# CIS565-Fall-2017/Project3-CUDA-Path-Tracer

Hardware: AMD Instinct MI355X
Metric: Mrays/sec (live paths x bounces) at 800x800 Cornell depth 8 (higher is better)
Workload: dtype f32

## Files before the change

project3-cuda-path-tracer_amd/csrc/pt_h_api.hpp:

```cpp
#pragma once

namespace one {

const char *pt_last_error(void) { return g_err; }
const char *pt_version(void) {
#ifdef PT_EXPERIMENTS
    return "ptmi355 0.1 (gfx950, fp32 no-contract, wave64) +experiments";
#else
    return "ptmi355 0.1 (gfx950, fp32 no-contract, wave64)";
#endif
}

void pt_free(void) {
    if (!R.live && !R.scratch) return;
    if (R.stream) (void)hipStreamSynchronize(R.stream);
    for (int k = 0; k < OV_MAX_LANES; ++k) {
        if (R.lane[k].stream) (void)hipStreamSynchronize(R.lane[k].stream);
        if (R.lane[k].la_stream) (void)hipStreamSynchronize(R.lane[k].la_stream);
    }
    if (R.la_gstream) (void)hipStreamSynchronize(R.la_gstream);
    for (int k = 0; k < 2; ++k) if (R.pool_mem[k]) (void)hipFree(R.pool_mem[k]);
    if (R.isect_mem) (void)hipFree(R.isect_mem);
    if (R.sort_table) (void)hipFree(R.sort_table);
    if (R.cache_mem) (void)hipFree(R.cache_mem);
    if (R.state_mem) (void)hipFree(R.state_mem);
    if (R.state_ended) (void)hipFree(R.state_ended);
    if (R.final_mem) (void)hipFree(R.final_mem);
    if (R.image && R.own_image) (void)hipFree(R.image);
    if (R.d_geoms) (void)hipFree(R.d_geoms);
    if (R.d_mats) (void)hipFree(R.d_mats);
    if (R.d_tris) (void)hipFree(R.d_tris);
    if (R.d_cull) (void)hipFree(R.d_cull);
    if (R.d_grec) (void)hipFree(R.d_grec);
    if (R.d_tri_bound) (void)hipFree(R.d_tri_bound);
    if (R.d_ginfo) (void)hipFree(R.d_ginfo);
    if (R.d_env) (void)hipFree(R.d_env);
    if (R.d_lights) (void)hipFree(R.d_lights);
    if (R.tex.d_texels) (void)hipFree(R.tex.d_texels);
    if (R.tex.d_tab) (void)hipFree(R.tex.d_tab);
    if (R.bump.d_texels) (void)hipFree(R.bump.d_texels);
    if (R.bump.d_tab) (void)hipFree(R.bump.d_tab);
    if (R.d_vnormals) (void)hipFree(R.d_vnormals);
    if (R.mesh_hit) (void)hipFree(R.mesh_hit);
    for (int k = 0; k < 2; ++k) if (R.mesh_flags[k]) (void)hipFree(R.mesh_flags[k]);
    if (R.d_bvh_nodes) (void)hipFree(R.d_bvh_nodes);
    if (R.d_bvh_meshes) (void)hipFree(R.d_bvh_meshes);
    if (R.d_bvh_tris) (void)hipFree(R.d_bvh_tris);
    if (R.d_bvh_top) (void)hipFree(R.d_bvh_top);
    if (R.d_cam_mask) (void)hipFree(R.d_cam_mask);
    R.d_cam_mask = nullptr; R.cam_mask_valid = false;
    if (R.d_cull0) (void)hipFree(R.d_cull0);
    R.d_cull0 = nullptr; R.cull0_tiles = 0;
    free_lanes();
    if (R.ctl) (void)hipFree(R.ctl);
    if (R.dir_mem) (void)hipFree(R.dir_mem);
// ... 155 lines not shown
    if (const char *wm = getenv("PTMI355_WHOLE_MAX_HOST")) R.whole_max_host_paths = strtoull(wm, nullptr, 10);
    if (getenv("PTMI355_WHOLE_MAX") && !getenv("PTMI355_WHOLE_MAX_HOST")) R.whole_max_host_paths = R.whole_max_paths;
    if (const char *e = getenv("PTMI355_OVERLAP")) {
        const int nl = atoi(e);
        R.ov_enabled = nl != 0;
        if (nl >= 2) { R.ov_lanes = std::min(nl, OV_MAX_LANES); R.ov_lanes_set = true; }
    }
    if (const char *e = getenv("PTMI355_OVERLAP_GB")) R.ov_budget_gb = atof(e);
    if (const char *e = pt_experiment("PTMI355_LANE_STREAMS")) R.ov_streams = std::max(1, atoi(e));
    R.epi_enabled = true;
    if (const char *e = pt_experiment("PTMI355_HOST_EPILOGUE")) R.epi_enabled = atoi(e) != 0;
    if (d->flags & PT_MOMENTS) R.epi_enabled = false;
    if (const char *e = pt_experiment("PTMI355_EPI_DIRECT")) R.epi_direct_enabled = atoi(e) != 0;
    R.defer_enabled = true;
    if (const char *e = pt_experiment("PTMI355_DEFER_DIR")) R.defer_enabled = atoi(e) != 0;
    R.own_enabled = true;
    if (const char *e = pt_experiment("PTMI355_OWN_SURFACE")) R.own_enabled = atoi(e) != 0;
    R.first_hit_enabled = true;
    if (const char *e = pt_experiment("PTMI355_FIRST_HIT")) R.first_hit_enabled = atoi(e) != 0;
    R.first_two_enabled = true;
    if (const char *e = pt_experiment("PTMI355_FIRST_TWO")) R.first_two_enabled = atoi(e) != 0;
    R.first_state_enabled = true;
    if (const char *e = pt_experiment("PTMI355_FIRST_STATE")) R.first_state_enabled = atoi(e) != 0;
    R.host_sparse_enabled = (d->flags & (PT_HOST_SPARSE | PT_SHARED_IMAGE)) != 0;
    if (const char *e = pt_experiment("PTMI355_ASYNC_DIRECT")) R.async_direct_enabled = atoi(e) != 0;
    R.pin_enabled = true;
    if (const char *e = pt_experiment("PTMI355_PIN")) R.pin_enabled = atoi(e) != 0;
    R.npix = W * H;
    R.map.W = W; R.map.H = H; R.map.tile_index = d->tile_index; R.map.tile_count = tile_count;
    R.map.strip_rows = tile_count > 1 ? d->strip_rows : H;
    R.map.tile_pixels = tile_rows(d->tile_index, tile_count, R.map.strip_rows, H) * W;
    if (R.map.tile_pixels <= 0) return fail(PT_ERR_INVALID, "pt_init: tile owns no rows");
    make_div_magic((uint32_t)R.map.tile_pixels, &R.map.div_magic, &R.map.div_shift);
    auto magic_holds = [](uint32_t d, uint32_t magic, uint32_t shift) {
        auto fast = [&](uint32_t n) {
            if (d == 1) return n;
            const uint32_t q = (uint32_t)(((uint64_t)magic * n) >> 32);
            return (((n - q) >> 1) + q) >> shift;
        };
        for (uint64_t k = 0; k <= 0xffffffffull / d && k < 4096; ++k)
            for (int e = -1; e <= 1; ++e) {
                const uint64_t n = k * d + (uint64_t)(int64_t)e;
                if (n <= 0xffffffffull && fast((uint32_t)n) != (uint32_t)n / d) return false;
            }
        const uint32_t probes[] = {0u, 1u, d - 1, d, d + 1, 0x7fffffffu, 0x80000000u, 0xfffffffeu, 0xffffffffu};
        for (uint32_t n : probes)
// ... 86 lines not shown
        if (d->num_materials >= (1 << 28)) return fail(PT_ERR_INVALID, "pt_init: at most 2^28 materials");
        HIPCHK(hipMalloc(&R.d_grec, gath.size() * 4));
        HIPCHK(hipMalloc((void **)&R.d_ginfo, ginfo.size() * 4));
        HIPCHK(hipMemcpy(R.d_grec, gath.data(), gath.size() * 4, hipMemcpyHostToDevice));
        HIPCHK(hipMemcpy(R.d_ginfo, ginfo.data(), ginfo.size() * 4, hipMemcpyHostToDevice));
        if (d->num_geoms > 0) {
            hipLaunchKernelGGL(k_face_normals, dim3((d->num_geoms * 8 + BLOCK - 1) / BLOCK), dim3(BLOCK), 0, R.stream,
                               R.d_grec, (const uint32_t *)R.d_ginfo, d->num_geoms);
            HIPCHK(hipGetLastError());
            HIPCHK(hipStreamSynchronize(R.stream));
        }
        R.scene.grec = R.d_grec; R.scene.ginfo = R.d_ginfo;
    }
    R.mesh_mode = MESH_NONE;
    for (int i = 0; i < d->num_geoms; ++i)
        if (d->geoms[i].type == PT_TRIANGLE_MESH) R.mesh_mode = (d->flags & PT_MESH_BVH) ? MESH_BVH : MESH_TILES;
    R.geoms_keep.assign(d->geoms, d->geoms + d->num_geoms);
    if (d->num_triangles > 0) R.tris_keep.assign(d->triangles, d->triangles + d->num_triangles);
    R.desc.geoms = R.geoms_keep.data();
    R.desc.triangles = R.tris_keep.empty() ? nullptr : R.tris_keep.data();
    if (d->num_meshes > 0) R.meshes_keep.assign(d->meshes, d->meshes + d->num_meshes);
    R.desc.meshes = R.meshes_keep.empty() ? nullptr : R.meshes_keep.data();
    R.grec_frames.assign((size_t)std::max(1, d->num_geoms) * 4, 0.0f);
    {
        const int rc = upload_cull(&R.desc, R.cam);
        if (rc != PT_OK) return rc;
    }
    if (R.mesh_mode == MESH_BVH) {
        const int rc = upload_bvh(&R.desc, grec);
        if (rc != PT_OK) return rc;
        HIPCHK(hipMemcpy(R.d_geoms, grec.data(), grec.size() * 4, hipMemcpyHostToDevice));
    }
    R.grec_keep = grec;
    {
        const size_t base = ((size_t)LDS_CTL_WORDS + (size_t)WAVES * PW_WORDS) * 4 +
                            (R.mesh_mode == MESH_TILES ? (size_t)WAVES * TRQ_WORDS * 4 : 0);
        const size_t scene = (size_t)scene_lds_words(d->num_materials, d->num_geoms) * 4;
        R.scene_lds = base + scene <= 32 * 1024;
        if (const char *e = getenv("PTMI355_SCENE_LDS")) R.scene_lds = atoi(e) != 0 && base + scene <= 64 * 1024;
        R.lds_bytes = base + (R.scene_lds ? scene : 0);
        R.lds_bytes = (R.lds_bytes + 15) & ~(size_t)15;
        if (const char *pad = pt_experiment("PTMI355_LDS_PAD")) R.lds_bytes += (size_t)atoi(pad);
    }

    R.sort_keys = 0;
    if ((R.flags & PT_SORT_MATERIAL) && (R.flags & PT_COMPACT) && !(R.flags & (PT_UNFUSED | PT_FAKE_SHADER | PT_CACHE_FIRST)) &&
// ... 60 lines not shown
    HIPCHK(hipMalloc((void **)&R.persist, sizeof(Persist)));
    HIPCHK(hipMemsetAsync(R.persist, 0, sizeof(Persist), R.stream));
    hipDeviceProp_t prop;
    HIPCHK(hipGetDeviceProperties(&prop, d->device));
    const int cus = prop.multiProcessorCount > 0 ? prop.multiProcessorCount : 256;
    int per_cu = 8;
    {
        const bool sorted = R.sort_keys > 0;
        const bool own = R.mesh_mode == MESH_NONE && !sorted;
        auto size_for = [&](auto sh) -> int {
            constexpr int SH = decltype(sh)::value;
            constexpr int SHN = SH & ~SH_SMOOTH;
            const void *fns[2];
            if (R.mesh_mode == MESH_BVH) { fns[0] = bounce_fn<MESH_PRE, SH>(R.scene_lds, false, false); fns[1] = bounce_fn<MESH_PRE, SH>(R.scene_lds, true, false); }
            else if (R.mesh_mode == MESH_TILES) { fns[0] = bounce_fn<MESH_TILES, SH>(R.scene_lds, false, sorted); fns[1] = bounce_fn<MESH_TILES, SH>(R.scene_lds, true, sorted); }
            else { fns[0] = bounce_fn<MESH_NONE, SHN>(R.scene_lds, false, sorted); fns[1] = bounce_fn<MESH_NONE, SHN>(R.scene_lds, true, sorted); }
            const void *fns_own[2] = {own ? bounce_fn<MESH_NONE, SHN>(R.scene_lds, false, false, true) : fns[0], own ? bounce_fn<MESH_NONE, SHN>(R.scene_lds, true, false, true) : fns[1]};
            const void *fns_tab[4] = {own ? bounce_fn<MESH_NONE, SHN>(R.scene_lds, false, false, false, true) : fns[0], own ? bounce_fn<MESH_NONE, SHN>(R.scene_lds, true, false, false, true) : fns[1],
                                      own ? bounce_fn<MESH_NONE, SHN>(R.scene_lds, false, false, true, true) : fns[0], own ? bounce_fn<MESH_NONE, SHN>(R.scene_lds, true, false, true, true) : fns[1]};
            const void *fns_two[2] = {own ? bounce_fn<MESH_NONE, SHN>(R.scene_lds, true, false, false, true, true) : fns[0],
                                      own ? bounce_fn<MESH_NONE, SHN>(R.scene_lds, true, false, true, true, true) : fns[0]};
            const void *fns_state[2] = {own ? bounce_fn<MESH_NONE, SHN>(R.scene_lds, true, false, false, true, true, true) : fns[0],
                                        own ? bounce_fn<MESH_NONE, SHN>(R.scene_lds, true, false, true, true, true, true) : fns[0]};
            for (const void *f : {fns[0], fns[1], fns_own[0], fns_own[1], fns_tab[0], fns_tab[1], fns_tab[2], fns_tab[3], fns_two[0], fns_two[1],
                                  fns_state[0], fns_state[1]}) {
                int n = 0;
                HIPCHK(hipOccupancyMaxActiveBlocksPerMultiprocessor(&n, f, BLOCK, R.lds_bytes));
                per_cu = std::min(per_cu, n);
            }
            return PT_OK;
        };
        int rc = size_for(std::integral_constant<int, 0>{});
        if (rc == PT_OK && (R.nlights > 0 || sky_session())) rc = size_for(std::integral_constant<int, SH_DIRECT>{});
        if (rc == PT_OK && (R.flags & PT_TEXTURES) && !(R.flags & PT_FAKE_SHADER)) rc = size_for(std::integral_constant<int, SH_TEX>{});
        if (rc == PT_OK && (R.flags & PT_SMOOTH_NORMALS) && !(R.flags & PT_FAKE_SHADER) && R.mesh_mode != MESH_NONE)
            rc = size_for(std::integral_constant<int, SH_SMOOTH>{});
        if (rc != PT_OK) return rc;
    }
    if (per_cu < 1) per_cu = 1;
    if (per_cu > 8) per_cu = 8;
    if (const char *e = pt_experiment("PTMI355_WGS_PER_CU")) per_cu = std::max(1, std::min(per_cu, atoi(e)));
    R.grid = (int)std::min<uint32_t>((R.max_tiles + WAVES - 1) / WAVES, (uint32_t)cus * (uint32_t)per_cu);
    R.per_cu = per_cu;
    if (const char *e = pt_experiment("PTMI355_LA_CUS")) R.la_cus = std::max(0, std::min(64, atoi(e) & ~7));
    if (R.grid < 1) R.grid = 1;
    if (R.grid * WAVES > 8192) R.grid = 8192 / WAVES;
    {
        int n = 0;
// ... 724 lines not shown
```

project3-cuda-path-tracer_amd/csrc/pt_h_enqueue.hpp:

```cpp
#pragma once

namespace {

BounceArgs bounce_args(int depth) {
    BounceArgs a{};
    a.dbg_counts = R.dbg_counts;
    a.in = R.pool[R.cur];
    a.out = (R.flags & PT_COMPACT) ? R.pool[R.cur ^ 1] : R.pool[R.cur];
    a.isect = R.isect;
    a.scene = R.scene;
    a.map = R.map;
    a.ctl = R.ctl;
    a.dir_in = tile_dir((R.flags & PT_COMPACT) ? R.cur_dir : -1);
    a.dir_out = tile_dir(depth);
    a.fin = R.final_mem;
    a.fin_stamp = R.fin_serial;
    a.cam = R.cam;
    a.lens = R.lens;
    a.depth = depth; a.trace_depth = R.trace_depth; a.iter0 = R.step_iter0;
    a.pool_n = (uint32_t)R.map.tile_pixels * (uint32_t)R.step_count;
    a.gen_rays = (depth == 0 && R.gen_fused) ? 1 : 0;
    a.mesh_hit = R.mesh_hit;
    a.mesh_flags_in = R.mesh_flags[depth & 1]; a.mesh_flags_out = R.mesh_flags[(depth + 1) & 1];
    a.mesh_scan = R.mesh_marked ? 0 : 1;
// ... 64 lines not shown
            if (R.mesh_mode == MESH_BVH) { constexpr int MESH = MESH_BVH; CALL; }            \
            else if (R.mesh_mode == MESH_TILES) { constexpr int MESH = MESH_TILES; CALL; }   \
            else { constexpr int MESH = MESH_NONE; CALL; }              \
        }                                                               \
    } while (0)

void launch_intersect(const Pool &in, const uint32_t *n_ptr, uint32_t n_fixed, const RangeDir &dir,
                      const uint32_t *nprev, bool raygen_pool = false, bool generate = false) {
    const bool same_rays = !R.lens.aa && !(R.lens.radius > 0.0f);
    const unsigned long long *cull0 = (raygen_pool && R.cull0_tiles && same_rays) ? R.d_cull0 : nullptr;
    RayGen gen{};
    if (generate) {
        gen.cam = R.cam; gen.lens = R.lens; gen.map = R.map; gen.trace_depth = R.trace_depth;
        gen.iter0 = R.step_iter0;
        PT_MESH_DISPATCH(hipLaunchKernelGGL((k_intersect<MESH, SLDS, true>), dim3(R.grid), dim3(BLOCK), R.lds_bytes, R.stream, in,
                                            R.isect, R.scene, n_ptr, n_fixed, dir, nprev, R.ctl, cull0, R.cull0_tiles, gen));
        return;
    }
    PT_MESH_DISPATCH(hipLaunchKernelGGL((k_intersect<MESH, SLDS>), dim3(R.grid), dim3(BLOCK), R.lds_bytes, R.stream, in,
                                        R.isect, R.scene, n_ptr, n_fixed, dir, nprev, R.ctl, cull0, R.cull0_tiles, gen));
}

template <int MESH, int SH = 0>
const void *bounce_fn(bool slds, bool gen, bool sorted, bool own = false, bool table = false, bool first2 = false, bool state2 = false) {
    if constexpr (MESH == MESH_NONE) {
        if (table && !sorted) {
            constexpr int SH0 = SH & (SH_ENV | SH_GLOSSY);
            if (first2 && state2) {
                if (own) return slds ? (const void *)k_bounce<MODE_STATE2, true, MESH, true, true, false, true, 0> : (const void *)k_bounce<MODE_STATE2, true, MESH, false, true, false, true, 0>;
                return slds ? (const void *)k_bounce<MODE_STATE2, true, MESH, true, true, false, false, 0> : (const void *)k_bounce<MODE_STATE2, true, MESH, false, true, false, false, 0>;
            }
            if (first2) {
                if (own) return slds ? (const void *)k_bounce<MODE_FIRST2, true, MESH, true, true, false, true, SH0> : (const void *)k_bounce<MODE_FIRST2, true, MESH, false, true, false, true, SH0>;
                return slds ? (const void *)k_bounce<MODE_FIRST2, true, MESH, true, true, false, false, SH0> : (const void *)k_bounce<MODE_FIRST2, true, MESH, false, true, false, false, SH0>;
            }
            if (own) {
                if (slds) return gen ? (const void *)k_bounce<MODE_CACHE0, true, MESH, true, true, false, true, SH0> : (const void *)k_bounce<MODE_CACHE0, true, MESH, true, false, false, true, SH0>;
                return gen ? (const void *)k_bounce<MODE_CACHE0, true, MESH, false, true, false, true, SH0> : (const void *)k_bounce<MODE_CACHE0, true, MESH, false, false, false, true, SH0>;
            }
            if (slds) return gen ? (const void *)k_bounce<MODE_CACHE0, true, MESH, true, true, false, false, SH0> : (const void *)k_bounce<MODE_CACHE0, true, MESH, true, false, false, false, SH0>;
            return gen ? (const void *)k_bounce<MODE_CACHE0, true, MESH, false, true, false, false, SH0> : (const void *)k_bounce<MODE_CACHE0, true, MESH, false, false, false, false, SH0>;
        }
        if (own && !sorted) {
            if (slds) return gen ? (const void *)k_bounce<MODE_FUSED, true, MESH, true, true, false, true, SH> : (const void *)k_bounce<MODE_FUSED, true, MESH, true, false, false, true, SH>;
            return gen ? (const void *)k_bounce<MODE_FUSED, true, MESH, false, true, false, true, SH> : (const void *)k_bounce<MODE_FUSED, true, MESH, false, false, false, true, SH>;
        }
    }
    if constexpr (MESH != MESH_PRE) {
// ... 124 lines not shown
        R.sorted_isects = true;
        R.step_depth = depth + 1;
        return PT_OK;
    }
    const bool same_rays = !R.lens.aa && !(R.lens.radius > 0.0f);
    const bool auto0 = depth == 0 && !unfused && R.first_hit_enabled && R.cache_mem != nullptr && !(R.flags & PT_FAKE_SHADER) &&
                       R.mesh_mode == MESH_NONE && R.sort_keys == 0 && same_rays && a.tex_tab == nullptr &&
                       !(a.nlights > 0 && depth >= a.trace_depth - 1);
    const bool cached0 = depth == 0 && !unfused && ((R.flags & PT_CACHE_FIRST) || auto0);
    const bool first2 = may_fuse && auto0 && !(R.flags & PT_CACHE_FIRST) && compact && R.gen_fused && R.first_two_enabled &&
                        R.trace_depth >= 2 && !(a.nlights > 0 && 1 >= a.trace_depth - 1);
    const bool state2 = first2 && R.state_mem != nullptr && a.env_n == 0;
    if (first2) {
        depth = 1;
        a.depth = 1;
        a.dir_out = tile_dir(1);
        a.gen_rays = 1;
    }
    a.defer_dir = (compact && !unfused && R.mesh_mode == MESH_NONE && R.sort_keys == 0 && depth + 1 < R.trace_depth &&
                   R.defer_enabled) ? 1 : 0;
    R.own_form = own_surface_plan((uint64_t)a.pool_n, R.scene.ngeoms,
                                  compact && !unfused && R.mesh_mode == MESH_NONE && R.sort_keys == 0 &&
                                  R.own_enabled);
    if (cached0 && !R.cache_valid) {
        StageTimer tm(PT_STAGE_INTERSECT);
        const Isect cache{R.cache_mem, (uint32_t)R.map.tile_pixels};
        const int blocks = std::min(R.grid, (R.map.tile_pixels + BLOCK - 1) / BLOCK);
        const hipStream_t fs = R.lane_cur ? R.lane_main : R.stream;
        PT_MESH_DISPATCH(hipLaunchKernelGGL((k_cache_first<MESH, SLDS>), dim3(blocks), dim3(BLOCK), R.lds_bytes, fs,
                                            cache, R.scene, R.cam, R.map, R.state_mem, R.state_ended));
        HIPCHK(hipGetLastError());
        if (R.lane_cur) {
            HIPCHK(hipEventRecord(R.ov_enter, fs));
            HIPCHK(hipStreamWaitEvent(R.stream, R.ov_enter, 0));
            R.first_hit_refence = true;
        }
        R.cache_valid = true;
        R.first_hit_fills++;
    }
    if (!cached0 && !unfused && R.mesh_mode == MESH_BVH) {
        StageTimer tm(PT_STAGE_MESH);
        if (compact) hipLaunchKernelGGL((k_mesh<true>), dim3(R.grid_mesh), dim3(MESH_BLOCK), MESH_LDS_BYTES, R.stream, a);
        else hipLaunchKernelGGL((k_mesh<false>), dim3(R.grid_mesh), dim3(MESH_BLOCK), MESH_LDS_BYTES, R.stream, a);
        HIPCHK(hipGetLastError());
    }
    StageTimer tm(PT_STAGE_BOUNCE);
    if (cached0) {
        a.isect = Isect{R.cache_mem, (uint32_t)R.map.tile_pixels};
        R.first_hit_launches++;
        if (state2) {
            a.first_state = R.state_mem; a.first_ended = R.state_ended; a.first_ended_tiles = (uint32_t)(R.map.tile_pixels / TILE);
            R.first_two_launches++; R.first_state_launches++; tm.two_bounces(); launch_bounce<MODE_STATE2, true>(a);
        }
        else if (first2) { R.first_two_launches++; tm.two_bounces(); launch_bounce<MODE_FIRST2, true>(a); }
        else if (compact) launch_bounce<MODE_CACHE0, true>(a); else launch_bounce<MODE_CACHE0, false>(a);
    } else if (unfused) {
        if (compact) launch_bounce<MODE_ISECT, true>(a); else launch_bounce<MODE_ISECT, false>(a);
    } else {
        if (compact) launch_bounce<MODE_FUSED, true>(a); else launch_bounce<MODE_FUSED, false>(a);
    }
    HIPCHK(hipGetLastError());
    if (R.mesh_mode == MESH_BVH) {
        R.mesh_marked = !cached0 && !unfused;
    }
    if (compact) { R.cur ^= 1; R.cur_dir = depth; }
    R.pool_own = R.own_form;
    R.step_depth = depth + 1;
    return PT_OK;
}

int enqueue_fake(void) {
    const uint32_t total = (uint32_t)R.map.tile_pixels * (uint32_t)R.step_count;
    launch_intersect(R.pool[R.cur], nullptr, total, tile_dir(-1), nullptr);
    HIPCHK(hipGetLastError());
    hipLaunchKernelGGL(k_shade_fake, dim3((total + BLOCK - 1) / BLOCK), dim3(BLOCK), 0, R.stream, R.pool[R.cur],
                       R.isect, R.scene.mats, R.map, R.step_iter0, total, R.final_mem, R.fin_serial);
    HIPCHK(hipGetLastError());
    R.step_depth = 1;
    return PT_OK;
}
// ... 270 lines not shown
```

project3-cuda-path-tracer_amd/csrc/pt_h_scene.hpp:

```cpp
#pragma once

namespace {

int upload_tri_bounds(const pt_scene_desc *d, double Rorigin);

int upload_cull(const pt_scene_desc *d, const pt_camera &cam) {
    const int n = d->num_geoms;
    std::vector<const float *> inv((size_t)std::max(1, n));
    std::vector<char> sph((size_t)std::max(1, n)), skip((size_t)std::max(1, n));
    for (int i = 0; i < n; ++i) {
        inv[(size_t)i] = &d->geoms[i].inverseTransform.m[0][0];
        sph[(size_t)i] = d->geoms[i].type == PT_SPHERE;
        skip[(size_t)i] = d->geoms[i].type == PT_TRIANGLE_MESH;
    }
    const double eye[3] = {(double)cam.position.x, (double)cam.position.y, (double)cam.position.z};
    std::vector<ptcull::Box> boxes;
    std::vector<double> pts(eye, eye + 3);
    for (int t = 0; t < d->num_triangles; ++t) {
        const pt_vec3 *v = &d->triangles[t].v0;
        double m = 0.0;
        for (int k = 0; k < 3; ++k) m = std::max(m, (double)std::fabs(v[k].x) + std::fabs(v[k].y) + std::fabs(v[k].z));
        if (t == 0 || m > pts[3]) { if (pts.size() < 6) pts.resize(6, 0.0); pts[3] = m; pts[4] = 0.0; pts[5] = 0.0; }
    }
    R.scene.rmax = ptcull::make_boxes(inv.data(), reinterpret_cast<const bool *>(sph.data()),
                                      reinterpret_cast<const bool *>(skip.data()), n, pts.data(), (int)(pts.size() / 3), boxes);
    std::vector<float> rec((size_t)std::max(1, n) * CULL_WORDS, 0.0f);
    for (int i = 0; i < n; ++i) {
        float *r = rec.data() + (size_t)i * CULL_WORDS;
        for (int k = 0; k < 3; ++k) ptcull::centre_half(boxes[(size_t)i].lo[k], boxes[(size_t)i].hi[k], r[2 * k], r[2 * k + 1]);
        int ax = 3;
        if (d->geoms[i].type == PT_CUBE && !pt_experiment("PTMI355_NO_AXIS_REJECT"))
            ax = ptcull::reject_row(&d->geoms[i].inverseTransform.m[0][0], &r[7]);
        if (ax == 4 && pt_experiment("PTMI355_NO_ROW_REJECT")) ax = 3;
        const int tw = d->geoms[i].type | (ax << 8);
        memcpy(&r[6], &tw, 4);
        const uint32_t ent = ((uint32_t)d->geoms[i].type << 7) | ((uint32_t)i << 9);
        memcpy(&r[11], &ent, 4);
    }
    if (!R.d_cull) HIPCHK(hipMalloc(&R.d_cull, rec.size() * 4));
    HIPCHK(hipMemcpyAsync(R.d_cull, rec.data(), rec.size() * 4, hipMemcpyHostToDevice, R.stream));
    HIPCHK(hipStreamSynchronize(R.stream));
    R.scene.cull = R.d_cull;
    R.cull_eye_reach = std::fabs(eye[0]) + std::fabs(eye[1]) + std::fabs(eye[2]);
    return upload_tri_bounds(d, (double)R.scene.rmax);
}

void make_tri_bounds(const pt_triangle *tris, int count, double Rorigin, float *out) {
    const double u = 0x1p-24;
    const float pad = ptbvh::spec_pad(reinterpret_cast<const float *>(tris), count);
    const int n4 = (count + 3) & ~3;
    for (int i = 0; i < n4; ++i) {
        float *o = out + (size_t)i * 4;
        if (i >= count) { o[0] = o[1] = o[2] = 0.0f; o[3] = -1.0f; continue; }
        const pt_triangle &t = tris[i];
        const float v0[3] = {t.v0.x, t.v0.y, t.v0.z};
        const float e1[3] = {t.v1.x - t.v0.x, t.v1.y - t.v0.y, t.v1.z - t.v0.z};
        const float e2[3] = {t.v2.x - t.v0.x, t.v2.y - t.v0.y, t.v2.z - t.v0.z};
        double c[3], h2 = 0.0, cinf = 0.0;
        bool fin = true;
        for (int a = 0; a < 3; ++a) {
            const float x1 = v0[a] + e1[a], x2 = v0[a] + e2[a];
            const float lo = std::fmin(v0[a], std::fmin(x1, x2)) - pad, hi = std::fmax(v0[a], std::fmax(x1, x2)) + pad;
            if (!std::isfinite(lo) || !std::isfinite(hi)) fin = false;
// ... 235 lines not shown
```

project3-cuda-path-tracer_amd/csrc/pt_h_session.hpp:

```cpp
#pragma once

namespace {

constexpr size_t ERR_BYTES = 512;
char g_err[ERR_BYTES] = "";
thread_local char *t_err = g_err;

int fail(int code, const char *fmt, ...) {
    va_list ap;
    va_start(ap, fmt);
    vsnprintf(t_err, ERR_BYTES, fmt, ap);
    va_end(ap);
    return code;
}

#define HIPCHK(expr)                                                                            \
    do {                                                                                        \
        hipError_t e_ = (expr);                                                                 \
        if (e_ != hipSuccess)                                                                   \
            return fail(PT_ERR_DEVICE, "HIP error (%s:%d): %s: %s", __builtin_strrchr(__FILE__, '/') ? __builtin_strrchr(__FILE__, '/') + 1 : __FILE__, __LINE__, #expr, \
                        hipGetErrorString(e_));                                                 \
    } while (0)

template <class Texel> struct CubeMaps {
// ... 13 lines not shown
    uint32_t flags = 0;
    int device = 0;
    hipStream_t stream = nullptr;
    bool own_stream = false;
    TileMap map{};
    int npix = 0;
    uint32_t cap = 0;
    int max_batch = 1;
    float *pool_mem[2] = {nullptr, nullptr};
    Pool pool[2]{};
    int cur = 0;
    float *isect_mem = nullptr;
    uint32_t *sort_table = nullptr;
    float *cache_mem = nullptr;
    bool cache_valid = false;
    bool first_hit_enabled = true;
    bool first_hit_refence = false;
    bool first_two_enabled = true;
    uint64_t first_two_launches = 0;
    float *state_mem = nullptr;
    uint32_t *state_ended = nullptr;
    bool first_state_enabled = true;
    uint64_t first_state_launches = 0;
    uint64_t first_hit_fills = 0, first_hit_launches = 0;
    Isect isect{};
    float *final_mem = nullptr;
    uint32_t fin_serial = 0;
    float *image = nullptr;
    bool own_image = false;
    float *d_geoms = nullptr, *d_mats = nullptr, *d_tris = nullptr;
    float *d_cull = nullptr, *d_grec = nullptr;
    float *d_tri_bound = nullptr;
    size_t tri_bound_words = 0;
    std::vector<float> grec_frames;
    uint32_t *d_ginfo = nullptr;
    double cull_eye_reach = 0.0;
    std::vector<pt_geom> geoms_keep;
    std::vector<pt_triangle> tris_keep;
    std::vector<pt_mesh> meshes_keep;
    std::vector<float> grec_keep;
    bool scene_lds = true;
    SceneDev scene{};
    float4 *d_env = nullptr;
    int env_n = 0;
    std::vector<float> env_keep;
    float *d_lights = nullptr;
// ... 249 lines not shown
```

project3-cuda-path-tracer_amd/csrc/pt_k_bounce.hpp:

```cpp
#pragma once

namespace {

enum { MODE_FUSED = 0, MODE_ISECT = 1, MODE_CACHE0 = 2, MODE_FIRST2 = 3, MODE_STATE2 = 4 };
constexpr bool mode_first2(int mode) { return mode == MODE_FIRST2 || mode == MODE_STATE2; }

template <typename T>
__device__ __forceinline__ T karg_field(size_t offset) {
    const __attribute__((address_space(4))) char *kp = (const __attribute__((address_space(4))) char *)__builtin_amdgcn_kernarg_segment_ptr();
    asm volatile("" : "+s"(kp));
    return *(const __attribute__((address_space(4))) T *)(kp + offset);
}
template <typename T>
__device__ __forceinline__ T karg_struct(size_t offset) {
    static_assert(sizeof(T) % 4 == 0, "whole dwords");
    const __attribute__((address_space(4))) char *kp = (const __attribute__((address_space(4))) char *)__builtin_amdgcn_kernarg_segment_ptr();
    asm volatile("" : "+s"(kp));
    uint32_t w[sizeof(T) / 4];
#pragma unroll
    for (size_t k = 0; k < sizeof(T) / 4; ++k) w[k] = *(const __attribute__((address_space(4))) uint32_t *)(kp + offset + 4 * k);
    T t;
    __builtin_memcpy(&t, w, sizeof(T));
    return t;
}
// ... 511 lines not shown
        asm volatile("s_waitcnt vmcnt(0)" ::: "memory");
        __syncthreads();
        if (threadIdx.x == 0) {
            const bool last = elect_last(a.ctl->bucket[a.depth][0], &a.ctl->done[a.depth]);
            if (last) {
                __builtin_amdgcn_fence(__ATOMIC_ACQUIRE, "agent");
                asm volatile("s_waitcnt vmcnt(0)" ::: "memory");
            }
            sctl[0] = last ? 1u : 0u;
        }
        __syncthreads();
        STAMP(7);
        if (sctl[0]) {
            const unsigned long long t0 = __builtin_amdgcn_s_memrealtime();
            scan_range_counts(a.dir_out, &a.ctl->nlive[a.depth + 1], sctl + 16, R * TILE, PT_ALIGNED_TILES && !SORT);
            if (threadIdx.x == 0) a.ctl->scan_ticks[a.depth] = (uint32_t)(__builtin_amdgcn_s_memrealtime() - t0);
#ifdef PT_STAMPS
            if (threadIdx.x == 0 && a.depth == PT_STAMPS) { a.ctl->stamp[8] = t0; a.ctl->stamp[9] = __builtin_amdgcn_s_memrealtime(); }
#endif
        }
    }
}

__device__ __forceinline__ void fold_iter_counts(const uint32_t *counts, uint32_t G, int depth, Control *ctl, Persist *per, HostStats *hs,
                                                 uint32_t iterations, uint32_t serial, uint32_t *lds ) {
    constexpr int PER_PASS = BLOCK / 32;
    unsigned long long rays = 0;
    uint32_t first = 0;
    for (int d0 = 0; d0 < depth; d0 += PER_PASS) {
        const int d = d0 + (int)(threadIdx.x >> 5);
        uint32_t sum = 0;
        if (d < depth)
            for (uint32_t b = threadIdx.x & 31u; b < G; b += 32u)
                sum += __hip_atomic_load(&counts[(uint32_t)d * G + b], __ATOMIC_RELAXED, __HIP_MEMORY_SCOPE_AGENT);
        for (int off = 16; off > 0; off >>= 1) sum += __shfl_down(sum, off, 32);
        if ((threadIdx.x & 31u) == 0) lds[threadIdx.x >> 5] = sum;
        __syncthreads();
        if (threadIdx.x == 0)
            for (int k = 0; k < PER_PASS && d0 + k < depth; ++k) {
                const uint32_t tot = lds[k];
                ctl->alive[d0 + k] = tot;
                if (hs) hs->alive[d0 + k] = tot;
                rays += tot;
                if (d0 + k == 0) first = tot;
            }
        __syncthreads();
// ... 134 lines not shown
```

project3-cuda-path-tracer_amd/csrc/pt_types.hpp:

```cpp
#pragma once

namespace {


#ifndef PT_MIN_WAVES
#define PT_MIN_WAVES 4
#endif
#ifndef PT_FUSED_WAVES
#define PT_FUSED_WAVES 6
#endif
#ifndef PT_ISECT_WAVES
#define PT_ISECT_WAVES 4
#endif
#ifndef PT_PRE_WAVES
#define PT_PRE_WAVES 6
#endif
#ifndef PT_ITER_WAVES
#define PT_ITER_WAVES PT_MIN_WAVES
#endif
#ifndef PT_SORT_WAVES
#define PT_SORT_WAVES 6
#endif
#ifndef PT_LOOP_WAVES
#define PT_LOOP_WAVES 3
// ... 203 lines not shown
    const unsigned long long *cam_mask;
    const unsigned long long *cull0;
    uint32_t cull0_tiles;
    float *epi_image, *epi_host;
    int epi_direct;
    uint32_t *iter_counts;
    Persist *persist;
    HostStats *host_stats;
    uint32_t *sort_table;
    int nbins;
    int defer_dir;
    const float4 *env;
    int env_n;
    const float *lights;
    int nlights;
    const float4 *tex;
    const int2 *tex_tab;
    const ptd::bump_texel *bumps;
    const int2 *bump_tab;
    float *first_state;
    const uint32_t *first_ended;
    uint32_t first_ended_tiles;
    const float *vnormals;
};

enum : uint32_t { FS_ZERO = 0, FS_CONST = 1, FS_DIFFUSE = 2, FS_FIXED = 3, FS_KIND_MASK = 3 };
__host__ __device__ constexpr size_t first_state_bytes(size_t tile_pixels) { return ((tile_pixels + 63) / 64) * 2560; }

enum : int {
    SH_ENV = 1,
    SH_GLOSSY = 2,
    SH_DIRECT = 4,
    SH_TEX = 8,
    SH_SMOOTH = 16
};

struct RayGen {
    pt_camera cam;
    Lens lens;
    TileMap map;
    int trace_depth, iter0;
};

__device__ __forceinline__ int local_to_pixel(const TileMap &m, int j) {
    if (m.tile_count == 1) return j;
    int ly = j / m.W;
    int x = j - ly * m.W;
// ... 38 lines not shown
```

project3-cuda-path-tracer_amd/csrc/ptmi355.hip:

```cpp
#include <hip/hip_runtime.h>

#include <algorithm>
#include <atomic>
#include <cfloat>
#include <cmath>
#include <cstdarg>
#include <cstdio>
#include <cstdlib>
#include <cstring>
#include <type_traits>
#include <vector>

#include "../../include/ptmi355.h"
#include "pt_device.hpp"

static_assert(sizeof(pt_vec3) == 12 && sizeof(pt_mat4) == 64 && sizeof(pt_ray) == 24, "ABI");
static_assert(sizeof(pt_geom) == 236 && offsetof(pt_geom, transform) == 44 &&
              offsetof(pt_geom, inverseTransform) == 108 && offsetof(pt_geom, invTranspose) == 172, "Geom ABI");
static_assert(sizeof(pt_material) == 44 && offsetof(pt_material, hasReflective) == 28 &&
              offsetof(pt_material, emittance) == 40, "Material ABI");
static_assert(sizeof(pt_camera) == 84 && offsetof(pt_camera, view) == 32 &&
              offsetof(pt_camera, pixelLength) == 76, "Camera ABI");
static_assert(sizeof(pt_path_segment) == 44 && offsetof(pt_path_segment, pixelIndex) == 36, "PathSegment ABI");
static_assert(sizeof(pt_shadeable_intersection) == 20 && offsetof(pt_shadeable_intersection, materialId) == 16,
// ... 77 lines not shown

extern "C" int ptdbg_first_two(unsigned long long out[1]) {
    if (G.live) {
        out[0] = 0;
        for (auto &wp : G.w) out[0] += wp->ctx.first_two_launches;
        return 0;
    }
    if (!g_single.live) return -1;
    out[0] = g_single.first_two_launches;
    return 0;
}

extern "C" int ptdbg_first_state(unsigned long long out[1]) {
    if (G.live) {
        out[0] = 0;
        for (auto &wp : G.w) out[0] += wp->ctx.first_state_launches;
        return 0;
    }
    if (!g_single.live) return -1;
    out[0] = g_single.first_state_launches;
    return 0;
}

extern "C" int ptdbg_denoise(unsigned long long out[3]) {
    if (!g_single.live) return -1;
    for (int k = 0; k < 3; ++k) out[k] = g_single.dn_launches[k];
    return 0;
}

extern "C" int ptdbg_denoise_times(const pt_denoise_params *params, int iter, int reps, float *ms) {
    if (G.live) return fail(PT_ERR_INVALID, "ptdbg_denoise_times: single-device sessions");
    return one::denoise_times(params, iter, reps, ms);
}

extern "C" int ptdbg_temporal(unsigned long long out[2]) {
    if (!g_single.live) return -1;
    for (int k = 0; k < 2; ++k) out[k] = g_single.tp_launches[k];
    return 0;
}

extern "C" int ptdbg_temporal_times(const pt_denoise_params *params, const pt_temporal_params *temporal, int iter, int reps, float *ms) {
    if (G.live) return fail(PT_ERR_INVALID, "ptdbg_temporal_times: single-device sessions");
    return one::temporal_times(params, temporal, iter, reps, ms);
}

extern "C" int ptdbg_variance(unsigned long long out[2]) {
// ... 30 lines not shown
```

Baseline: 65330.

## Add last-bounce kernel that traces only rays aimed at emitter boxes

Adds a specialized kernel for the final bounce. It first culls each ray against the bounding boxes of the emissive primitives and compacts only the rays that could hit a light into dense 64-lane batches for full intersection and shading. Rays that cannot reach an emitter are dropped, because they contribute nothing at the last bounce. This removes most intersection work at the final depth, at the cost of extra ballot/compaction logic, a new kernel variant that may lower the occupancy minimum, and a correctness dependence on the cull boxes being conservative.

```diff
diff --git a/profiles/last_aimed/count_aimed.py b/profiles/last_aimed/count_aimed.py
--- /dev/null
+++ b/profiles/last_aimed/count_aimed.py
@@ -0,0 +1,58 @@
+import os
+import sys
+
+import numpy as np
+
+ROOT = os.path.dirname(os.path.dirname(os.path.dirname(os.path.abspath(__file__))))
+sys.path.insert(0, ROOT)
+sys.path.insert(0, os.path.join(ROOT, "tests"))
+
+import __graft_entry__ as ge
+import cull_model
+
+
+def main(argv):
+    pt = ge.load_package()
+    pt.build_host()
+    from oracle import pyoracle as po
+    po.build(ref=False)
+    scn = pt.load_scene(argv[0] if argv else os.path.join(ROOT, "scenes", "cornell.txt"))
+    cam = scn.camera.copy()
+    if len(argv) >= 3:
+        w, h = int(argv[1]), int(argv[2])
+        cam["resolution"][0] = (w, h)
+        ys = np.tan(np.float32(cam["fov"][0][1]) * np.float32(np.pi / 180))
+        xs = np.float32(ys * np.float32(w) / np.float32(h))
+        cam["pixelLength"][0] = (np.float32(2 * xs / np.float32(w)), np.float32(2 * ys / np.float32(h)))
+    geoms, mats, depth = scn.geoms, scn.materials, scn.traceDepth
+    ref = po.Tracer(np.ascontiguousarray(geoms).view(po.GEOM_DT), mats.view(po.MATERIAL_DT), cam, depth, flags=po.F_COMPACT, trig=po.TRIG_SHARED)
+    snaps = []
+    ref.iterate(1, snapshots=snaps)
+    eye = tuple(float(x) for x in np.asarray(cam["position"]).reshape(-1)[:3])
+    boxes, rmax, _ = pt.cull_boxes(geoms, eye)
+    lit = [g for g in range(len(geoms)) if mats["emittance"][geoms["materialid"][g]] > 0]
+    print("%s %dx%d depth %d, emissive primitives %s" % (os.path.basename(argv[0]) if argv else "cornell.txt", cam["resolution"][0][0], cam["resolution"][0][1], depth, lit))
+    print("| rays entering bounce | rays | aimed | nearest hit emissive | aimed lanes per 64-tile | tiles with no aimed lane |")
+    print("|---|---|---|---|---|---|")
+    for d in range(1, len(snaps)):
+        n = snaps[d]["n_before"]
+        p = snaps[d - 1]["paths"][:n]
+        assert snaps[d - 1]["n_live"] == n and (p["remainingBounces"] > 0).all()
+        rays = np.concatenate([p["origin"], p["direction"]], axis=1).astype(np.float32)
+        aimed = np.zeros(n, bool)
+        for e in lit:
+            cand, wild = cull_model.candidates(rays, boxes[e].reshape(2, 3), rmax, None)
+            aimed |= cand | wild
+        isects = snaps[d]["isects"][:n]
+        hit = isects["t"] > 0
+        emissive = hit & (mats["emittance"][np.where(hit, isects["materialId"], 0)] > 0)
+        assert not (emissive & ~aimed).any(), "bounce %d: an emissive nearest hit outside every emissive box" % d
+        pad = np.zeros((n + 63) // 64 * 64, bool)
+        pad[:n] = aimed
+        per_tile = pad.reshape(-1, 64).sum(axis=1)
+        print("| %d%s | %d | %.2f %% | %.2f %% | %.2f | %.1f %% |" % (d, " (the last)" if d == depth - 1 else "", n, 100 * aimed.mean(), 100 * emissive.mean(),
+                                                                 per_tile.mean(), 100 * (per_tile == 0).mean()))
+
+
+if __name__ == "__main__":
+    main(sys.argv[1:])
diff --git a/project3-cuda-path-tracer_amd/csrc/pt_h_api.hpp b/project3-cuda-path-tracer_amd/csrc/pt_h_api.hpp
--- a/project3-cuda-path-tracer_amd/csrc/pt_h_api.hpp
+++ b/project3-cuda-path-tracer_amd/csrc/pt_h_api.hpp
@@ -31,6 +31,7 @@
     if (R.d_mats) (void)hipFree(R.d_mats);
     if (R.d_tris) (void)hipFree(R.d_tris);
     if (R.d_cull) (void)hipFree(R.d_cull);
+    if (R.d_emit_cull) (void)hipFree(R.d_emit_cull);
     if (R.d_grec) (void)hipFree(R.d_grec);
     if (R.d_tri_bound) (void)hipFree(R.d_tri_bound);
     if (R.d_ginfo) (void)hipFree(R.d_ginfo);
@@ -232,6 +233,8 @@
     if (const char *e = pt_experiment("PTMI355_FIRST_TWO")) R.first_two_enabled = atoi(e) != 0;
     R.first_state_enabled = true;
     if (const char *e = pt_experiment("PTMI355_FIRST_STATE")) R.first_state_enabled = atoi(e) != 0;
+    R.last_aimed_enabled = true;
+    if (const char *e = pt_experiment("PTMI355_LAST_AIMED")) R.last_aimed_enabled = atoi(e) != 0;
     R.host_sparse_enabled = (d->flags & (PT_HOST_SPARSE | PT_SHARED_IMAGE)) != 0;
     if (const char *e = pt_experiment("PTMI355_ASYNC_DIRECT")) R.async_direct_enabled = atoi(e) != 0;
     R.pin_enabled = true;
@@ -364,6 +367,8 @@
     if (d->num_meshes > 0) R.meshes_keep.assign(d->meshes, d->meshes + d->num_meshes);
     R.desc.meshes = R.meshes_keep.empty() ? nullptr : R.meshes_keep.data();
     R.grec_frames.assign((size_t)std::max(1, d->num_geoms) * 4, 0.0f);
+    for (int i = 0; i < d->num_geoms; ++i)
+        if (d->materials[d->geoms[i].materialid].emittance > 0.0f) R.emit_geoms.push_back(i);
     {
         const int rc = upload_cull(&R.desc, R.cam);
         if (rc != PT_OK) return rc;
@@ -470,8 +475,10 @@
                                       own ? bounce_fn<MESH_NONE, SHN>(R.scene_lds, true, false, true, true, true) : fns[0]};
             const void *fns_state[2] = {own ? bounce_fn<MESH_NONE, SHN>(R.scene_lds, true, false, false, true, true, true) : fns[0],
                                         own ? bounce_fn<MESH_NONE, SHN>(R.scene_lds, true, false, true, true, true, true) : fns[0]};
+            const void *fns_last[2] = {own ? bounce_fn<MESH_NONE, SHN>(R.scene_lds, false, false, false, false, false, false, true) : fns[0],
+                                       own ? bounce_fn<MESH_NONE, SHN>(R.scene_lds, false, false, true, false, false, false, true) : fns[0]};
             for (const void *f : {fns[0], fns[1], fns_own[0], fns_own[1], fns_tab[0], fns_tab[1], fns_tab[2], fns_tab[3], fns_two[0], fns_two[1],
-                                  fns_state[0], fns_state[1]}) {
+                                  fns_state[0], fns_state[1], fns_last[0], fns_last[1]}) {
                 int n = 0;
                 HIPCHK(hipOccupancyMaxActiveBlocksPerMultiprocessor(&n, f, BLOCK, R.lds_bytes));
                 per_cu = std::min(per_cu, n);
diff --git a/project3-cuda-path-tracer_amd/csrc/pt_h_enqueue.hpp b/project3-cuda-path-tracer_amd/csrc/pt_h_enqueue.hpp
--- a/project3-cuda-path-tracer_amd/csrc/pt_h_enqueue.hpp
+++ b/project3-cuda-path-tracer_amd/csrc/pt_h_enqueue.hpp
@@ -110,8 +110,13 @@
 }
 
 template <int MESH, int SH = 0>
-const void *bounce_fn(bool slds, bool gen, bool sorted, bool own = false, bool table = false, bool first2 = false, bool state2 = false) {
+const void *bounce_fn(bool slds, bool gen, bool sorted, bool own = false, bool table = false, bool first2 = false, bool state2 = false,
+                      bool last = false) {
     if constexpr (MESH == MESH_NONE) {
+        if (last && !gen && !sorted && !table) {
+            if (own) return slds ? (const void *)k_bounce_last<true, true> : (const void *)k_bounce_last<false, true>;
+            return slds ? (const void *)k_bounce_last<true, false> : (const void *)k_bounce_last<false, false>;
+        }
         if (table && !sorted) {
             constexpr int SH0 = SH & (SH_ENV | SH_GLOSSY);
             if (first2 && state2) {
@@ -282,6 +287,10 @@
     R.own_form = own_surface_plan((uint64_t)a.pool_n, R.scene.ngeoms,
                                   compact && !unfused && R.mesh_mode == MESH_NONE && R.sort_keys == 0 &&
                                   R.own_enabled);
+    const bool last_aimed = may_fuse && R.last_aimed_enabled && depth >= 1 && depth == R.trace_depth - 1 && compact && !unfused && !cached0 &&
+                            !a.gen_rays && R.mesh_mode == MESH_NONE && R.sort_keys == 0 && !(R.flags & (PT_GLOSSY | PT_FAKE_SHADER)) &&
+                            a.env_n == 0 && a.nlights == 0 && a.tex_tab == nullptr && a.vnormals == nullptr &&
+                            (int)R.emit_geoms.size() <= LAST_MAX_EMITTERS;
     if (cached0 && !R.cache_valid) {
         StageTimer tm(PT_STAGE_INTERSECT);
         const Isect cache{R.cache_mem, (uint32_t)R.map.tile_pixels};
@@ -316,6 +325,16 @@
         else if (compact) launch_bounce<MODE_CACHE0, true>(a); else launch_bounce<MODE_CACHE0, false>(a);
     } else if (unfused) {
         if (compact) launch_bounce<MODE_ISECT, true>(a); else launch_bounce<MODE_ISECT, false>(a);
+    } else if (last_aimed) {
+        a.emit_cull = R.d_emit_cull; a.emit_n = (int)R.emit_geoms.size();
+        R.last_aimed_launches++;
+        if (R.own_form) {
+            if (R.scene_lds) hipLaunchKernelGGL((k_bounce_last<true, true>), dim3(R.grid), dim3(BLOCK), R.lds_bytes, R.stream, a);
+            else hipLaunchKernelGGL((k_bounce_last<false, true>), dim3(R.grid), dim3(BLOCK), R.lds_bytes, R.stream, a);
+        } else {
+            if (R.scene_lds) hipLaunchKernelGGL((k_bounce_last<true, false>), dim3(R.grid), dim3(BLOCK), R.lds_bytes, R.stream, a);
+            else hipLaunchKernelGGL((k_bounce_last<false, false>), dim3(R.grid), dim3(BLOCK), R.lds_bytes, R.stream, a);
+        }
     } else {
         if (compact) launch_bounce<MODE_FUSED, true>(a); else launch_bounce<MODE_FUSED, false>(a);
     }
diff --git a/project3-cuda-path-tracer_amd/csrc/pt_h_scene.hpp b/project3-cuda-path-tracer_amd/csrc/pt_h_scene.hpp
--- a/project3-cuda-path-tracer_amd/csrc/pt_h_scene.hpp
+++ b/project3-cuda-path-tracer_amd/csrc/pt_h_scene.hpp
@@ -39,6 +39,11 @@
     }
     if (!R.d_cull) HIPCHK(hipMalloc(&R.d_cull, rec.size() * 4));
     HIPCHK(hipMemcpyAsync(R.d_cull, rec.data(), rec.size() * 4, hipMemcpyHostToDevice, R.stream));
+    std::vector<float> erec(std::max<size_t>(1, R.emit_geoms.size()) * CULL_WORDS, 0.0f);
+    for (size_t k = 0; k < R.emit_geoms.size(); ++k)
+        memcpy(erec.data() + k * CULL_WORDS, rec.data() + (size_t)R.emit_geoms[k] * CULL_WORDS, CULL_WORDS * 4);
+    if (!R.d_emit_cull) HIPCHK(hipMalloc(&R.d_emit_cull, erec.size() * 4));
+    HIPCHK(hipMemcpyAsync(R.d_emit_cull, erec.data(), erec.size() * 4, hipMemcpyHostToDevice, R.stream));
     HIPCHK(hipStreamSynchronize(R.stream));
     R.scene.cull = R.d_cull;
     R.cull_eye_reach = std::fabs(eye[0]) + std::fabs(eye[1]) + std::fabs(eye[2]);
diff --git a/project3-cuda-path-tracer_amd/csrc/pt_h_session.hpp b/project3-cuda-path-tracer_amd/csrc/pt_h_session.hpp
--- a/project3-cuda-path-tracer_amd/csrc/pt_h_session.hpp
+++ b/project3-cuda-path-tracer_amd/csrc/pt_h_session.hpp
@@ -59,6 +59,10 @@
     uint32_t *state_ended = nullptr;
     bool first_state_enabled = true;
     uint64_t first_state_launches = 0;
+    std::vector<int> emit_geoms;
+    float *d_emit_cull = nullptr;
+    bool last_aimed_enabled = true;
+    uint64_t last_aimed_launches = 0;
     uint64_t first_hit_fills = 0, first_hit_launches = 0;
     Isect isect{};
     float *final_mem = nullptr;
diff --git a/project3-cuda-path-tracer_amd/csrc/pt_k_bounce.hpp b/project3-cuda-path-tracer_amd/csrc/pt_k_bounce.hpp
--- a/project3-cuda-path-tracer_amd/csrc/pt_k_bounce.hpp
+++ b/project3-cuda-path-tracer_amd/csrc/pt_k_bounce.hpp
@@ -557,6 +557,140 @@
     }
 }
 
+struct LastQ {
+    float *ray, *col;
+    uint32_t *pid;
+    uint32_t n;
+};
+
+template <bool OWN>
+__device__ __forceinline__ void last_dense_tile(const BounceArgs &a, const TileCtx &c, WaveQ &q, LastQ &lq, int depth) {
+    const int lane = c.lane;
+    __builtin_amdgcn_fence(__ATOMIC_ACQ_REL, "wavefront");
+    const bool act = (uint32_t)lane < lq.n;
+    f3 ro = ptd::mk(0, 0, 0), rd = ptd::mk(0, 0, 1);
+    uint32_t own = 0u;
+    if (act) {
+        const float *ry = lq.ray + lane;
+        ro = ptd::mk(ry[0], ry[64], ry[128]);
+        rd = ptd::mk(ry[192], ry[256], ry[320]);
+        if (OWN) own = (lq.pid[lane] & OWN_MASK) >> OWN_SHIFT;
+    }
+    MeshBest mb;
+    cull_scene<MESH_NONE, OWN>(a.scene, c.acc, q, 0, nullptr, act, ro, rd, mb, nullptr, false, 0,
+                               OWN ? own_surface_miss(c.acc, own, ro, rd) : 0xffffffffu);
+    drain_to(q, c.acc, q.total);
+    if (act) {
+        float t; f3 nrm; int mat, outside, geom;
+        tile_result(q, 0, c.acc, a.scene.tris, mb, t, nrm, mat, outside, geom);
+        const float *cl = lq.col + lane;
+        ptd::PathState ps;
+        ps.o = ro; ps.d = rd; ps.c = ptd::mk(cl[0], cl[64], cl[128]);
+        bool deferred = false;
+        ptd::shade_scatter<false>(ps, t, nrm, mat, outside, c.acc.mats, 0, 0, depth, true, false, &deferred, nullptr);
+        put_final(karg_field<float *>(offsetof(BounceArgs, fin)), lq.pid[lane] & ~OWN_MASK, ps.c, c.stamp);
+    }
+    lq.n = 0;
+    __builtin_amdgcn_fence(__ATOMIC_ACQ_REL, "wavefront");
+}
+
+template <bool OWN>
+__device__ __forceinline__ void run_tiles_last(const BounceArgs &a, const TileCtx &c, WaveQ &q, int depth, uint32_t first_tile,
+                                               uint32_t count, uint32_t tiles, uint32_t n, bool packed_in, uint32_t span_in,
+                                               uint32_t &cur, bool aligned) {
+    const int lane = c.lane;
+    LastQ lq{q.rays(1), q.win(1), reinterpret_cast<uint32_t *>(q.best(1)), 0u};
+    cfloat *const ec = as_const(a.emit_cull);
+    cfloat *const ec_end = ec + a.emit_n * CULL_WORDS;
+    for (uint32_t r = 0; r < count; ++r) {
+        const uint32_t tile = first_tile + r;
+        if (tile >= tiles) break;
+        rotate_priority(r + (uint32_t)depth, PT_MIN_WAVES + 1);
+        bool active = false;
+        uint32_t src = 0;
+        if (aligned) {
+            const uint32_t *tb = a.dir_in.tbase();
+            while (tile >= tb[cur + 1]) ++cur;
+            const uint32_t t64 = (tile - tb[cur]) * TILE + (uint32_t)lane;
+            active = t64 < a.dir_in.count()[cur];
+            src = cur * span_in + t64;
+        } else {
+            const uint32_t i = tile * TILE + lane;
+            active = i < n;
+            src = i;
+            if (packed_in) src = resolve_src(a.dir_in, span_in, cur, i, active, a.ctl);
+        }
+        uint32_t pidw = DEAD_PID;
+        f3 ro = ptd::mk(0, 0, 0), rd = ptd::mk(0, 0, 1);
+        if (active) {
+            const SlotPtr p = karg_pool(offsetof(BounceArgs, in)).slot(src);
+            pidw = ppid(p);
+            ro = ptd::mk(pf(p, 0), pf(p, 1), pf(p, 2));
+            rd = ptd::mk(pf(p, 3), pf(p, 4), pf(p, 5));
+            if (pidw == DEAD_PID) active = false;
+        }
+        const bool pending = active && (pidw & PENDING_DIR) != 0u;
+        if (active) pidw &= ~PENDING_DIR;
+        if (pending) {
+            const uint32_t pid = OWN ? pidw & ~OWN_MASK : pidw;
+            const uint32_t smp = sample_of(a.map, pid);
+            const int pixel = local_to_pixel(a.map, (int)(pid - smp * (uint32_t)a.map.tile_pixels));
+            uint32_t rng = ptd::seeded_engine(c.iter0 + (int)smp, pixel, depth - 1);
+            rd = ptd::hemisphere(rd, rng);
+        }
+        const CullRay cr = cull_ray(ro, rd, a.scene.rmax);
+        uint64_t m = ballot64(cr.wild);
+        for (cfloat *cc = ec; cc != ec_end; cc += CULL_WORDS) {
+            float cb[6];
+#pragma unroll
+            for (int k = 0; k < 6; ++k) cb[k] = cc[k];
+            m |= ballot64(cull_box(cr, cb[0], cb[1], cb[2], cb[3], cb[4], cb[5]));
+        }
+        m &= ballot64(active);
+        if (m == 0) continue;
+        const uint32_t add = (uint32_t)__popcll((unsigned long long)m);
+        if (lq.n + add > 64u) last_dense_tile<OWN>(a, c, q, lq, depth);
+        if (lane_of(m)) {
+            const SlotPtr p = karg_pool(offsetof(BounceArgs, in)).slot(src);
+            const uint32_t s = lq.n + rank_below(m);
+            float *ry = lq.ray + s;
+            ry[0] = ro.x; ry[64] = ro.y; ry[128] = ro.z; ry[192] = rd.x; ry[256] = rd.y; ry[320] = rd.z;
+            float *cl = lq.col + s;
+            cl[0] = pf(p, 6); cl[64] = pf(p, 7); cl[128] = pf(p, 8);
+            lq.pid[s] = pidw;
+        }
+        lq.n += add;
+    }
+    if (lq.n) last_dense_tile<OWN>(a, c, q, lq, depth);
+}
+
+template <bool SLDS, bool OWN>
+__global__ __launch_bounds__(BLOCK, PT_FUSED_WAVES > PT_MIN_WAVES ? PT_FUSED_WAVES : PT_MIN_WAVES) void k_bounce_last(BounceArgs a) {
+    extern __shared__ __attribute__((aligned(16))) float lds_raw[];
+    const LdsCarve lc = carve_lds(lds_raw, a.scene, SLDS);
+    TileCtx c;
+    c.kargs = true;
+    c.tri_lds = nullptr;
+    c.acc = stage_scene<SLDS>(lc.scene, a.scene);
+    WaveQ q{lc.pw, 0, 0};
+    c.lane = threadIdx.x & 63;
+    const uint32_t W = gridDim.x * WAVES;
+    const uint32_t wid = run_id();
+    c.iter0 = a.iter0;
+    c.stamp = a.fin_stamp;
+    const uint32_t n = a.ctl->nlive[a.depth];
+    const bool packed_in = a.dir_in.mem != nullptr;
+    const bool aligned = PT_ALIGNED_TILES && packed_in;
+    const uint32_t tiles = aligned ? a.dir_in.tbase()[a.dir_in.nr] : (n + TILE - 1) / TILE;
+    const uint32_t R = (tiles + W - 1) / W;
+    const uint32_t span_in = packed_in ? *a.dir_in.span() : 0;
+    uint32_t cur = 0;
+    if (packed_in && wid * R < tiles)
+        cur = aligned ? find_range(a.dir_in.tbase(), a.dir_in.nr, wid * R) : find_range(a.dir_in.base(), a.dir_in.nr, wid * R * TILE);
+    run_tiles_last<OWN>(a, c, q, a.depth, wid * R, R, tiles, n, packed_in, span_in, cur, aligned);
+    if (blockIdx.x == 0 && threadIdx.x == 0) a.ctl->alive[a.depth] = n;
+}
+
 __device__ __forceinline__ void fold_iter_counts(const uint32_t *counts, uint32_t G, int depth, Control *ctl, Persist *per, HostStats *hs,
                                                  uint32_t iterations, uint32_t serial, uint32_t *lds ) {
     constexpr int PER_PASS = BLOCK / 32;
diff --git a/project3-cuda-path-tracer_amd/csrc/pt_types.hpp b/project3-cuda-path-tracer_amd/csrc/pt_types.hpp
--- a/project3-cuda-path-tracer_amd/csrc/pt_types.hpp
+++ b/project3-cuda-path-tracer_amd/csrc/pt_types.hpp
@@ -249,7 +249,10 @@
     const uint32_t *first_ended;
     uint32_t first_ended_tiles;
     const float *vnormals;
-};
+    const float *emit_cull;
+    int emit_n;
+};
+constexpr int LAST_MAX_EMITTERS = 8;
 
 enum : uint32_t { FS_ZERO = 0, FS_CONST = 1, FS_DIFFUSE = 2, FS_FIXED = 3, FS_KIND_MASK = 3 };
 __host__ __device__ constexpr size_t first_state_bytes(size_t tile_pixels) { return ((tile_pixels + 63) / 64) * 2560; }
diff --git a/project3-cuda-path-tracer_amd/csrc/ptmi355.hip b/project3-cuda-path-tracer_amd/csrc/ptmi355.hip
--- a/project3-cuda-path-tracer_amd/csrc/ptmi355.hip
+++ b/project3-cuda-path-tracer_amd/csrc/ptmi355.hip
@@ -123,6 +123,17 @@
     return 0;
 }
 
+extern "C" int ptdbg_last_aimed(unsigned long long out[1]) {
+    if (G.live) {
+        out[0] = 0;
+        for (auto &wp : G.w) out[0] += wp->ctx.last_aimed_launches;
+        return 0;
+    }
+    if (!g_single.live) return -1;
+    out[0] = g_single.last_aimed_launches;
+    return 0;
+}
+
 extern "C" int ptdbg_denoise(unsigned long long out[3]) {
     if (!g_single.live) return -1;
     for (int k = 0; k < 3; ++k) out[k] = g_single.dn_launches[k];
```

Measured after the change: 63690. -2.5%, worse.
